# sparisi/pvr_habitat

Measured on AMD Instinct MI355X. Metric: frames/sec embedded (ResNet50, 256x256), higher is better.
Workload: dtype f16; 1 GPU; configs[1]: ResNet50 (MoCo-v2 layout) frozen, 256x256 uint8 frames resident in HBM, batch 256/GPU, random-init synthetic weights, f16 storage / MFMA inputs with fp32 accumulation (the product default, inside the 1e-3 parity bound; configs[1] names bf16); global_batch=256, frame=256, chunk=256, batches_in_flight=2, parallelism=frame shards, no collective (dp1)

## Files before the change

### pvr_habitat_amd/csrc/bottleneck_chain.hip

```cpp
#include "encoder_internal.h"

namespace pvr {


__device__ __forceinline__ void ch_dma16(__amdgpu_buffer_rsrc_t rs, char *lds, int voff, int soff) {
    __builtin_amdgcn_raw_ptr_buffer_load_lds(rs, (__attribute__((address_space(3))) void *)lds, 16, voff, soff, 0, 0);
}

#ifdef CHAIN_STAMP
__device__ unsigned long long chain_stamps[8192][12];
#define CH_T(i_) { if (threadIdx.x == 0) ch_tt[i_] = __builtin_amdgcn_s_memrealtime(); }
#else
#define CH_T(i_)
#endif

#ifndef CH_KNOCK
#define CH_KNOCK 0
#endif
template <int AUX = 0>
__device__ __forceinline__ void store_b128_imm(u32x4 v, __amdgpu_buffer_rsrc_t rs, int voff, int imm) {
    if constexpr (!(CH_KNOCK & 1)) __builtin_amdgcn_raw_buffer_store_b128(v, rs, voff + imm, 0, AUX);
}

template <int CM, int CMN, bool F16, int RD, int OCC, bool HALO, bool DS = false, int PFK = -1>
__global__ __launch_bounds__(256, OCC) void bottleneck_chain_kernel(ChainP p) {
    typedef typename HT<F16>::V8 V8;
    constexpr int BM = 128, BK = 64, BN = CM;
    constexpr int A_CH = BM / 32, B_CH = BN / 32, TM = 4, TN = BN / 32;
    constexpr int KS = CM / 64, HROWS = CM == 64 ? 256 : 192, RL = CM == 64 ? 3 : 2;
    constexpr int HSL = HROWS * 128, RING_OFF = KS * HSL, SLICE = CM * 128, ZERO_OFF = (HROWS - 1) * 128;
    constexpr int HOPS = KS * HROWS / 32;
    constexpr int STAGE = HALO ? (RING_OFF + 2 * SLICE) / 2 : (BM + BN) * 128;
    constexpr int C4 = 4 * CM, G = C4 / 64, KS3 = CM / 64;
    constexpr int TN1 = CMN / 32;
    constexpr int W3_CH = CM / 32, W1_CH = CMN / 32;
    constexpr int T2_OFF = 0;
    constexpr int YG_OFF = KS3 * 16384;
    constexpr int W3_OFF = YG_OFF + 16384;
    constexpr int W1_OFF = W3_OFF + KS3 * 8192;
    static_assert(W3_OFF + KS3 * 8192 <= 2 * STAGE, "phase-B tiles must fit the phase-A area");
    static_assert(RD >= 1 && RD <= G, "residual prefetch depth");
    extern __shared__ __attribute__((aligned(16))) char smem[];

    const int tid = threadIdx.x, lane = tid & 63, wave = tid >> 6;
#ifdef CHAIN_STAMP
    unsigned long long ch_tt[12] = {0, 0, 0, 0, 0, 0, 0, 0, 0, 0, 0, 0};
#endif
    CH_T(0);
    const int m0 = xcd_remap(blockIdx.x, gridDim.x) * BM;
    const int srow = tid >> 3, pch = tid & 7;
    const auto rs_in = __builtin_amdgcn_make_buffer_rsrc(const_cast<u16 *>(p.in), 0, p.in_bytes, 0x00020000);
    const auto rs_w2 = __builtin_amdgcn_make_buffer_rsrc(const_cast<u16 *>(p.w2), 0, p.w2_bytes, 0x00020000);
    const auto rs_w3 = __builtin_amdgcn_make_buffer_rsrc(const_cast<u16 *>(p.w3), 0, p.w3_bytes, 0x00020000);
    const auto rs_w1 = __builtin_amdgcn_make_buffer_rsrc(const_cast<u16 *>(p.w1n), 0, p.w1n_bytes, 0x00020000);
    const auto rs_res = __builtin_amdgcn_make_buffer_rsrc(const_cast<u16 *>(DS ? p.xds : p.res), 0, DS ? p.xds_bytes : p.y_bytes, 0x00020000);
    const auto rs_wd = __builtin_amdgcn_make_buffer_rsrc(const_cast<u16 *>(DS ? p.wds : p.w3), 0, DS ? p.wds_bytes : p.w3_bytes, 0x00020000);
    const auto rs_y = __builtin_amdgcn_make_buffer_rsrc(p.y, 0, p.y_bytes, 0x00020000);
    const auto rs_t = __builtin_amdgcn_make_buffer_rsrc(p.t1n, 0, p.t1n_bytes, 0x00020000);
// ... 64 lines not shown

    const int wm = wave >> 1, wn = wave & 1;
    const int fr = lane & 15, fq = lane >> 4;
    int x_rd[2][TM];
    int b_rd[2][TN];
#pragma unroll
    for (int ks = 0; ks < 2; ++ks) {
#pragma unroll
        for (int j = 0; j < TM; ++j) {
            const int row = wm * 64 + j * 16 + fr;
            x_rd[ks][j] = row * 128 + (((ks * 4 + fq) ^ ((row >> 1) & 7)) << 4);
        }
#pragma unroll
        for (int i = 0; i < TN; ++i) {
            const int row = wn * (BN / 2) + i * 16 + fr;
            b_rd[ks][i] = BM * 128 + row * 128 + (((ks * 4 + fq) ^ ((row >> 1) & 7)) << 4);
        }
    }

    const int y_nhwc = ((m0 + wm * 64 + fr) * C4 + wn * 32 + fq * 8) * 2;
    const int y_blkd = ((m0 >> 4) + wm * 4) * (C4 * 32) + (wn * 4 + fq) * 256 + fr * 16;
    const int y_off0 = p.y_blk ? y_blkd : y_nhwc, y_js = p.y_blk ? C4 * 32 : 16 * C4 * 2, y_gs = p.y_blk ? 2048 : 128;
    const int r_off0 = p.res_blk ? y_blkd : y_nhwc, r_js = p.res_blk ? C4 * 32 : 16 * C4 * 2, r_gs = p.res_blk ? 2048 : 128;
    const int t_nhwc = ((m0 + wm * 64 + fr) * CMN + wn * (CMN / 2) + fq * 8) * 2;
    const int t_blkd = ((m0 >> 4) + wm * 4) * (CMN * 32) + (wn * (CMN / 16) + fq) * 256 + fr * 16;
    const int t_off0 = p.t_blk ? t_blkd : t_nhwc, t_js = p.t_blk ? CMN * 32 : 16 * CMN * 2;
#define Y_OFF(j_) (y_off0 + (j_) * y_js)
#define R_OFF(j_) (r_off0 + (j_) * r_js)
#define T_OFF(j_) (t_off0 + (j_) * t_js)
    const int st_r = tid >> 3, st_c = ((tid & 7) ^ ((st_r >> 1) & 7)) * 16;
    const int w3_g0 = st_r * CM * 2 + st_c, w3_l0 = W3_OFF + st_r * 128 + (tid & 7) * 16;
    const int w1_g0 = st_r * C4 * 2 + st_c, w1_l0 = W1_OFF + st_r * 128 + (tid & 7) * 16;
#define W3_G(i_) (w3_g0 + ((i_) & 1) * (32 * CM * 2) + ((i_) >> 1) * 128)
#define W3_L(i_) (w3_l0 + ((i_) & 1) * 4096 + ((i_) >> 1) * 8192)
#define W1_G(i_) (w1_g0 + (i_) * (32 * C4 * 2))
#define W1_L(i_) (w1_l0 + (i_) * 4096)
    u32x4 rres[RD][TM], w3r[W3_CH], w1r[CMN ? W1_CH : 1];
#define PVR_PHASE_B_PREFETCH()                                                                                          \
    {                                                                                                                   \
        if constexpr (!DS) {                                                                                            \
            _Pragma("unroll") for (int d = 0; d < RD; ++d)                                                              \
                _Pragma("unroll") for (int j = 0; j < TM; ++j)                                                          \
                    rres[d][j] = __builtin_bit_cast(u32x4, __builtin_amdgcn_raw_buffer_load_b128(rs_res, (CH_KNOCK & 2) ? OOB : R_OFF(j), d * r_gs, DS ? 0 : PVR_NT_AUX(16))); \
        }                                                                                                               \
        _Pragma("unroll") for (int i = 0; i < W3_CH; ++i)                                                               \
            w3r[i] = __builtin_bit_cast(u32x4, __builtin_amdgcn_raw_buffer_load_b128(rs_w3, W3_G(i), 0, 0));            \
        if constexpr (CMN > 0) {                                                                                        \
// ... 125 lines not shown
        const int c = wn * (BN / 2) + i * 16 + fq * 4;
        const float4 bv = *reinterpret_cast<const float4 *>(p.b2 + c);
#pragma unroll
        for (int j = 0; j < TM; ++j) {
            const int row = wm * 64 + j * 16 + fr;
            const f32x4 a = acc2[i][j];
            const unsigned lo = pack2_h<F16>(fmaxf(a[0] + bv.x, 0.f), fmaxf(a[1] + bv.y, 0.f));
            const unsigned hi = pack2_h<F16>(fmaxf(a[2] + bv.z, 0.f), fmaxf(a[3] + bv.w, 0.f));
            const int cc = c & 63;
            char *dst = smem + T2_OFF + (c >> 6) * 16384 + row * 128 + ((((cc >> 3) ^ ((row >> 1) & 7))) << 4) + (cc & 4) * 2;
            *reinterpret_cast<uint2 *>(dst) = make_uint2(lo, hi);
        }
    }
#pragma unroll
    for (int i = 0; i < W3_CH; ++i) *reinterpret_cast<u32x4 *>(smem + W3_L(i)) = w3r[i];
    if constexpr (CMN > 0) {
#pragma unroll
        for (int i = 0; i < W1_CH; ++i) *reinterpret_cast<u32x4 *>(smem + W1_L(i)) = w1r[i];
    }
    if (G > 1) {
#pragma unroll
        for (int i = 0; i < W3_CH; ++i)
            w3r[i] = __builtin_bit_cast(u32x4, __builtin_amdgcn_raw_buffer_load_b128(rs_w3, W3_G(i), 64 * CM * 2, 0));
        if constexpr (CMN > 0) {
#pragma unroll
            for (int i = 0; i < W1_CH; ++i) w1r[i] = __builtin_bit_cast(u32x4, __builtin_amdgcn_raw_buffer_load_b128(rs_w1, W1_G(i), 128, 0));
        }
    }
    __syncthreads();
    CH_T(3);

    int w3_rd[2][2], w1_rd[2][CMN ? TN1 : 1], yg_wr[TM];
#pragma unroll
    for (int ks = 0; ks < 2; ++ks) {
#pragma unroll
        for (int t = 0; t < 2; ++t) {
            const int row = wn * 32 + t * 16 + fr;
            w3_rd[ks][t] = W3_OFF + row * 128 + (((ks * 4 + fq) ^ ((row >> 1) & 7)) << 4);
        }
        if constexpr (CMN > 0) {
#pragma unroll
            for (int i = 0; i < TN1; ++i) {
                const int row = wn * (CMN / 2) + i * 16 + fr;
                w1_rd[ks][i] = W1_OFF + row * 128 + (((ks * 4 + fq) ^ ((row >> 1) & 7)) << 4);
            }
        }
    }
#pragma unroll
    for (int j = 0; j < TM; ++j) {
        const int row = wm * 64 + j * 16 + fr;
        yg_wr[j] = YG_OFF + row * 128 + (((wn * 4 + fq) ^ ((row >> 1) & 7)) << 4);
    }
    f32x4 acc1[CMN ? TN1 : 1][TM];
    if constexpr (CMN > 0) {
#pragma unroll
        for (int i = 0; i < TN1; ++i)
#pragma unroll
            for (int j = 0; j < TM; ++j) acc1[i][j] = f32x4{0.f, 0.f, 0.f, 0.f};
    }

#pragma unroll
    for (int g = 0; g < G; ++g) {
        if (g == 1) CH_T(6);
        f32x4 acc3[2][TM];
#pragma unroll
        for (int t = 0; t < 2; ++t)
// ... 52 lines not shown
            if (p.y_blk) store_b128_imm<PVR_NT_AUX(4)>(o, rs_y, Y_OFF(j) + g * y_gs, 0);
            else store_b128_imm(o, rs_y, Y_OFF(j) + g * y_gs, 0);
            if constexpr (CMN > 0) *reinterpret_cast<u32x4 *>(smem + yg_wr[j]) = o;
        }
        if (!DS && g + RD < G) {
#pragma unroll
            for (int j = 0; j < TM; ++j)
                rres[g % RD][j] = __builtin_bit_cast(u32x4, __builtin_amdgcn_raw_buffer_load_b128(rs_res, (CH_KNOCK & 2) ? OOB : R_OFF(j), (g + RD) * r_gs, DS ? 0 : PVR_NT_AUX(16)));
        }
        if (g == 1) CH_T(8);
        __syncthreads();
        if (g == 1) CH_T(9);
        if (g + 1 < G) {
#pragma unroll
            for (int i = 0; i < W3_CH; ++i) *reinterpret_cast<u32x4 *>(smem + W3_L(i)) = w3r[i];
            if (g + 2 < G) {
#pragma unroll
                for (int i = 0; i < W3_CH; ++i)
                    w3r[i] = __builtin_bit_cast(u32x4, __builtin_amdgcn_raw_buffer_load_b128(rs_w3, W3_G(i), (g + 2) * (64 * CM * 2), 0));
            }
        }
        if (g == 1) CH_T(10);
        if constexpr (CMN == 0) __syncthreads();
        if constexpr (CMN > 0) {
#pragma unroll
            for (int ks = 0; ks < 2; ++ks) {
                V8 xa[TM], wb[TN1];
#pragma unroll
                for (int j = 0; j < TM; ++j) xa[j] = *reinterpret_cast<const V8 *>(smem + YG_OFF + x_rd[ks][j]);
#pragma unroll
                for (int i = 0; i < TN1; ++i) wb[i] = *reinterpret_cast<const V8 *>(smem + w1_rd[ks][i]);
#pragma unroll
                for (int i = 0; i < TN1; ++i)
#pragma unroll
                    for (int j = 0; j < TM; ++j) acc1[i][j] = mfma16<F16>(wb[i], xa[j], acc1[i][j]);
            }
            __syncthreads();
            if (g == 1) CH_T(11);
            if (g + 1 < G) {
#pragma unroll
                for (int i = 0; i < W1_CH; ++i) *reinterpret_cast<u32x4 *>(smem + W1_L(i)) = w1r[i];
                if (g + 2 < G) {
#pragma unroll
                    for (int i = 0; i < W1_CH; ++i)
                        w1r[i] = __builtin_bit_cast(u32x4, __builtin_amdgcn_raw_buffer_load_b128(rs_w1, W1_G(i), (g + 2) * 128, 0));
                }
            }
        }
    }

    CH_T(4);
    if constexpr (CMN > 0) {
#pragma unroll
        for (int q = 0; q < TN1 / 2; ++q) {
            const int c0 = wn * (CMN / 2) + q * 32 + fq * 8;
            const float4 bA = *reinterpret_cast<const float4 *>(p.b1n + c0), bB = *reinterpret_cast<const float4 *>(p.b1n + c0 + 4);
#pragma unroll
            for (int j = 0; j < TM; ++j) {
                const f32x4 lo = acc1[2 * q][j], hi = acc1[2 * q + 1][j];
                const float v[8] = {lo[0] + bA.x, lo[1] + bA.y, lo[2] + bA.z, lo[3] + bA.w, hi[0] + bB.x, hi[1] + bB.y, hi[2] + bB.z, hi[3] + bB.w};
                u32x4 o;
#pragma unroll
                for (int e = 0; e < 4; ++e)
                    o[e] = pack2_h<F16>(fmaxf(v[2 * e], 0.f), fmaxf(v[2 * e + 1], 0.f));
                if (p.t_blk) store_b128_imm<0>(o, rs_t, T_OFF(j) + q * 1024, 0);
                else store_b128_imm<PVR_NT_AUX(8)>(o, rs_t, T_OFF(j), q * 64);
            }
        }
    }
#undef PVR_PHASE_B_PREFETCH
#undef W3_G
#undef W3_L
#undef W1_G
#undef W1_L
#undef Y_OFF
#undef R_OFF
#undef T_OFF
#ifdef CHAIN_STAMP
    CH_T(5);
    if (threadIdx.x == 0 && blockIdx.x < 8192) { _Pragma("unroll") for (int k = 0; k < 12; ++k) chain_stamps[blockIdx.x][k] = ch_tt[k]; }
#endif
}

template <int CM, int CMN, bool F16, int RD, int OCC, bool HALO, bool DS = false, int PFK = -1>
static pvr_status launch_chain_one(ChainP &p, hipStream_t stream) {
    const int grid = (p.M + 127) / 128;
    const size_t pipe = HALO ? (size_t)(CM / 64) * (CM == 64 ? 256 : 192) * 128 + (size_t)2 * CM * 128 : (size_t)2 * (128 + CM) * 128;
    const size_t phase_b = (CM / 64) * 16384 + 16384 + (CM / 64) * 8192 + CMN * 128;
    const size_t lds = phase_b <= pipe ? pipe : phase_b;
    static DeviceOnce attr_done;
    if (attr_done.needed()) {
        PVR_HIP_TRY(hipFuncSetAttribute((const void *)bottleneck_chain_kernel<CM, CMN, F16, RD, OCC, HALO, DS, PFK>,
                                        hipFuncAttributeMaxDynamicSharedMemorySize, (int)lds));
        attr_done.mark();
    }
    hipLaunchKernelGGL((bottleneck_chain_kernel<CM, CMN, F16, RD, OCC, HALO, DS, PFK>), dim3(grid), dim3(256), lds, stream, p);
    PVR_LAUNCH_CHECK();
    return PVR_OK;
}

template <int CM, int CMN, bool F16, int RD, int OCC, bool DS = false>
static pvr_status launch_chain_inst(ChainP &p, const PlanSwitches &sw, hipStream_t stream) {
    const bool halo = p.stride == 1 && 128 + 2 * p.W + 2 <= (CM == 64 ? 256 : 192) - 1 && sw.chain_halo;
    if constexpr (DS) {
        if (halo) return sw.chain_ds_occ == 3 ? launch_chain_one<CM, CMN, F16, RD, 3, true, true>(p, stream) : launch_chain_one<CM, CMN, F16, RD, 2, true, true>(p, stream);
        return launch_chain_one<CM, CMN, F16, RD, 2, false, true>(p, stream);
    } else {
        if (halo) {
            if constexpr (CM == 128) {
                if (sw.chain_pfk == 12) return launch_chain_one<CM, CMN, F16, RD, 2, true, false, 12>(p, stream);
            }
            return launch_chain_one<CM, CMN, F16, RD, (CM == 64 ? OCC : 2), true>(p, stream);
        }
        return launch_chain_one<CM, CMN, F16, RD, OCC, false>(p, stream);
    }
}

template <bool F16>
static pvr_status launch_chain_dt(ChainP &p, int cm, int cmn, const PlanSwitches &sw, hipStream_t stream) {
    if (p.xds) {
        if (cm == 64 && cmn == 64) return launch_chain_inst<64, 64, F16, 1, 2, true>(p, sw, stream);
        set_error("bottleneck chain with downsample: no instance for Cm=%d, next Cm=%d", cm, cmn);
        return PVR_ERR_INVALID;
    }
    const int cfg = sw.chain_cfg;
#define PVR_CHAIN64(CMN_)                                                                 \
    switch (cfg) {                                                                        \
    case 12: return launch_chain_inst<64, CMN_, F16, 1, 2>(p, sw, stream);                \
    case 13: return launch_chain_inst<64, CMN_, F16, 1, 3>(p, sw, stream);                \
    case 22: return launch_chain_inst<64, CMN_, F16, 2, 2>(p, sw, stream);                \
    case 23: return launch_chain_inst<64, CMN_, F16, 2, 3>(p, sw, stream);                \
    default: return launch_chain_inst<64, CMN_, F16, 4, 2>(p, sw, stream);                \
    }
    if (cm == 64 && cmn == 64) PVR_CHAIN64(64)
    if (cm == 64 && cmn == 128) {
        if (cfg / 10 == 1) return launch_chain_inst<64, 128, F16, 1, 2>(p, sw, stream);
        if (cfg / 10 == 2) return launch_chain_inst<64, 128, F16, 2, 2>(p, sw, stream);
        return launch_chain_inst<64, 128, F16, 4, 2>(p, sw, stream);
    }
    if (cm == 64 && cmn == 0) PVR_CHAIN64(0)
#undef PVR_CHAIN64
    if (cm == 128 && cmn == 128) return launch_chain_inst<128, 128, F16, 1, 2>(p, sw, stream);
    if (cm == 128 && cmn == 0) return launch_chain_inst<128, 0, F16, 1, 2>(p, sw, stream);
    set_error("bottleneck chain: no instance for Cm=%d, next Cm=%d", cm, cmn);
    return PVR_ERR_INVALID;
}

bool chain_uses_wave_form(const PlanSwitches &sw, int cm, int cmn, int stride, bool ds) { return sw.chain_wave && chain_wave_supported(sw, cm, cmn, stride, ds); }

bool chain_uses_wave128(const PlanSwitches &sw, int cm, int cmn, int stride, int64_t M) { return sw.chain_wave && chain_wave128_supported(sw, cm, cmn, stride, M); }

bool chain_ds_supported(int cm, int cmn, int cin, int stride) { return cm == 64 && cmn == 64 && cin == 64 && stride == 1; }
bool chain_supported(int cm, int cmn) { return (cm == 64 && (cmn == 0 || cmn == 64 || cmn == 128)) || (cm == 128 && (cmn == 0 || cmn == 128)); }

int chain_row_source(int row) { return (row & ~31) + 8 * ((row >> 2) & 3) + 4 * ((row >> 4) & 1) + (row & 3); }

pvr_status launch_bottleneck_chain(const PlanSwitches &sw, const void *t1, const void *w2, const float *b2, const void *w3p, const float *b3, const void *res,
                                   void *y, const void *w1np, const float *b1n, void *t1n, int n, int h, int w, int cm, int cmn,
                                   int stride, int dtype, hipStream_t stream, const void *xds, const void *wdsp, const void *w3pb, const void *wdspb,
                                   int wave, int in_blk, int out_blk, const void *wpk, int y_s2) {
    PVR_REQUIRE(chain_supported(cm, cmn), "bottleneck chain: unsupported widths Cm=%d next=%d", cm, cmn);
    PVR_REQUIRE(t1 && w2 && b2 && w3p && b3 && (res || xds) && y && (cmn == 0 || (w1np && b1n && t1n)), "bottleneck chain: null argument");
    PVR_REQUIRE(!xds || (wdsp && chain_ds_supported(cm, cmn, 64, stride)), "bottleneck chain with downsample: unsupported shape");
    ChainP p;
    p.in = (const u16 *)t1; p.w2 = (const u16 *)w2; p.w3 = (const u16 *)w3p; p.w1n = (const u16 *)w1np; p.res = (const u16 *)res;
    p.b2 = b2; p.b3 = b3; p.b1n = b1n; p.y = (u16 *)y; p.t1n = (u16 *)t1n;
    p.N = n; p.H = h; p.W = w; p.stride = stride;
    p.Ho = (h + 2 - 3) / stride + 1; p.Wo = (w + 2 - 3) / stride + 1;
    const int64_t M = (int64_t)n * p.Ho * p.Wo;
    const int64_t inb = (int64_t)n * h * w * cm * 2, yb = M * 4 * cm * 2, tb = M * (cmn ? cmn : 1) * 2;
    PVR_REQUIRE(inb < 0x7ffffff0ll && yb < 0x7ffffff0ll && tb < 0x7ffffff0ll, "bottleneck chain: operand larger than 2 GiB (use a smaller chunk)");
    p.M = (int)M; p.in_bytes = (unsigned)inb; p.y_bytes = (unsigned)yb; p.t1n_bytes = (unsigned)tb;
    p.xds = (const u16 *)xds; p.wds = (const u16 *)wdsp;
    p.xds_bytes = xds ? (unsigned)(M * 64 * 2) : 0; p.wds_bytes = xds ? (unsigned)(4 * cm * 64 * 2) : 0;
    p.w2_bytes = (unsigned)(cm * 9 * cm * 2); p.w3_bytes = (unsigned)(4 * cm * cm * 2); p.w1n_bytes = (unsigned)(cmn * 4 * cm * 2);
    if (wave == 2) {
// ... 18 lines not shown
```

### pvr_habitat_amd/csrc/encoder.hip

```cpp
#include "encoder_internal.h"

namespace pvr {

pvr_status launch_split16_pack(const float *w, void *out, int rows, int K, hipStream_t stream);
bool conv_split16_supported(int cin, int cout, int k);
pvr_status launch_conv_split16(const float *in, const void *wsp, const float *bias, const float *res, float *out, int n, int h, int w, int cin,
                               int cout, int k, int stride, int pad, int relu, hipStream_t stream, float *out2 = nullptr, int n1 = 0, void *out16 = nullptr,
                               int terms = 3);

void read_switches(PlanSwitches &sw) {
    auto get = [](const char *name, int def) { const char *v = getenv(name); return v ? atoi(v) : def; };
    sw.pool_fuse = get("PVR_POOL_FUSE", 1);
    sw.stem_u8 = get("PVR_STEM_U8", 1);
    sw.stem_lds = get("PVR_STEM_LDS", 1);
    sw.stem_regpool = get("PVR_STEM_REGPOOL", 1);
    sw.frame_front1 = get("PVR_FRAME_FRONT1", 1);
    sw.frame_next1 = get("PVR_FRAME_NEXT1", 0);
    sw.frame_bneck = get("PVR_FRAME_BNECK", 1);
    sw.frame64 = get("PVR_FRAME64", 0);
    sw.bneck_stagger = get("PVR_FRAME_STAGGER", 0);
    sw.dual_ds = get("PVR_DUAL_DS", 1);
    sw.chain_ds = get("PVR_CHAIN_DS", 1);
    sw.chain_blocked = get("PVR_CHAIN_BLOCKED", 1);
    sw.chain_halo = get("PVR_CHAIN_HALO", 1);
    sw.chain_ds_occ = get("PVR_CHAIN_DS_OCC", 3);
    sw.chain_pfk = get("PVR_CHAIN_PFK", 12);
    sw.chain_cfg = get("PVR_CHAIN_CFG", 12);
    sw.chain_wave = get("PVR_CHAIN_WAVE", 1);
    sw.chain_wave_halo = get("PVR_CHAIN_WAVE_HALO", 1);
    sw.chain_wave_128 = get("PVR_CHAIN_WAVE_128", 1);
    sw.strided_y = get("PVR_STRIDED_Y", 1);
    sw.chain_wave_l2 = get("PVR_CHAIN_WAVE_L2", 0);
    sw.splitk = get("PVR_SPLITK", 1);
    sw.smallk_div = get("PVR_SMALLK_DIV", 4);
    if (sw.smallk_div < 1) sw.smallk_div = 1;
    sw.frame_min_n = get("PVR_FRAME_MIN_N", 128);
    sw.frame_run = get("PVR_FRAME_RUN", 0);
    sw.frame_stagger = get("PVR_FRAME_RUN_STAGGER", 0);
    sw.split16 = get("PVR_SPLIT16", 1);
    sw.stem_conv1 = get("PVR_STEM_CONV1", 1);
    sw.resid32 = get("PVR_RESID32", 1);
    sw.tail_f32 = get("PVR_TAIL_F32", 1);
    sw.fuse = get("PVR_FUSE", 1);
    sw.conv_algo = get("PVR_CONV_ALGO", -1);
    sw.conv_halo = get("PVR_CONV_HALO", 1);
    sw.conv_expand = get("PVR_CONV_EXPAND", 1);
    sw.conv_wfrag = get("PVR_CONV_WFRAG", 1);
    sw.wfrag_ko = get("PVR_WFRAG_KO", 0);
    sw.igemm_nk4 = get("PVR_IGEMM_NK4", 1);
    sw.igemm_bm64 = get("PVR_IGEMM_BM64", 0);
    sw.pp_bm224 = get("PVR_PP_BM224", 1);
    sw.pp_persist = get("PVR_PP_PERSIST", 384);
}

// ... 552 lines not shown
        const int a_cmn = e->ops[A.next1].cout;
        if (!e->sw.chain_blocked) continue;
        if (B.t1_in != A.t1_out || b3.res_buf != a3.out_buf || !a3.tap.empty() || b2.h != a2.h / a2.stride || b2.w != a2.w / a2.stride || b2.stride != 1) continue;
        if (B.wave == 2) {
            A.out_blk = A.wave == 2 ? 1 : 3; B.in_blk = 1;
            continue;
        }
        if (!A.wave && !B.wave) {
            if ((b2.h * b2.w) % 16 == 0) { A.out_blk = 1; B.in_blk = 1; }
            continue;
        }
        if (!A.wave || !B.wave) continue;
        if (!chain_wave_blocked_ok(a_cmn, a2.h, a2.w)) continue;
        A.out_blk = 1; B.in_blk = 1;
        if (A.ds >= 0 && a > 0 && a2.w == 56 && e->sw.chain_wave_halo) {
            Launch &C = e->sched_fused[a - 1];
            if (C.conv3 < 0 && C.conv2 >= 0) {
                const ConvOp &c1 = e->ops[C.conv2];
                if (c1.kind == 0 && !c1.f32op && c1.k == 1 && c1.stride == 1 && c1.out_buf == A.t1_in && c1.tap.empty() && c1.res_buf == B_NONE && !c1.out_f32 &&
                    c1.ksplit <= 1) { C.out_blk = 1; A.in_blk = 1; }
            }
        }
    }
    if (e->sw.stem_conv1 && !e->sched_fused.empty() && (e->desc.arch == PVR_ARCH_RESNET50 || e->desc.arch == PVR_ARCH_RESNET50_L3 || e->desc.arch == PVR_ARCH_RESNET50_L4)) {
        const Launch &L0 = e->sched_fused[0];
        if (L0.conv3 < 0 && L0.ds < 0 && L0.pair < 0 && !L0.frame && L0.conv2 == 0) {
            const ConvOp &c1 = e->ops[0];
            if (c1.kind == 0 && !c1.f32op && !c1.from32 && c1.k == 1 && c1.stride == 1 && c1.cin == 64 && c1.cout == 64 && c1.cin_real == 64 && c1.cout_real == 64 && c1.relu == 1 &&
                c1.in_buf == B_X0 && c1.out_buf == B_T1 && c1.res_buf == B_NONE && !c1.out_f32 && c1.tap.empty() && c1.ksplit <= 1 && c1.h == 56 && (int)c1.h_w.size() == 64 * 64) {
                std::vector<u16> img(64 * 64);
                stem_c1_pack(c1.h_w.data(), img.data());
                pvr_status s = enc_upload(&e->d_stem_c1w, img);
                if (s) return s;
                e->stem_c1 = 0; e->stem_c1_blk = L0.out_blk;
                e->sched_fused.erase(e->sched_fused.begin());
            }
        }
    }
    if (e->sw.strided_y) {
        std::vector<Launch> &sc = e->sched_fused;
        for (size_t a = 0; a < sc.size(); ++a) {
            Launch &A = sc[a];
            if (A.conv3 < 0 || A.frame || A.wave != 1 || A.next1 < 0 || A.ds >= 0) continue;
            const ConvOp &a2 = e->ops[A.conv2], &a3 = e->ops[A.conv3];
            if (a2.stride != 1 || !chain_wave_y_s2_ok(a2.cout, e->ops[A.next1].cout, a2.h, a2.w, A.out_blk)) continue;
            const int yb = a3.out_buf;
// ... 454 lines not shown
            } else
                s = launch_conv(enc->sw, enc->d_buf[c1.in_buf], c1.d_w, c1.d_b, nullptr, enc->d_buf[c1.out_buf], enc->d_zero, nb, c1.h, c1.w, c1.cin, c1.cout, 1, 1, 1, 0, c1.relu, 0, dt, st);
            if (s) return s;
        }
        bool pooled = false;
        const std::vector<Launch> &plan_ = cur_plan(enc);
        const uint8_t *kinds = enc->kinds.data() + (size_t)(nb - 1) * plan_.size();
        float *smallk = enc->d_smallk[enc->cur_lane];
        const bool pool_args_ok = enc->stop_after.empty() && out_stride % 4 == 0 && (((size_t)(out + (size_t)f0 * out_stride)) & 15) == 0;
        int launch_idx = 0;
        const bool run_ok = enc->stop_after.empty() && !enc->range_flags;
        const int stop_idx = enc->stop_after.size() > 1 && enc->stop_after[0] == '#' ? atoi(enc->stop_after.c_str() + 1) : -1;
        auto member = [&](const ConvOp &o, const void *in, const void *r_, void *out_) -> pvr_status {
            if (const int ks = small_batch_ksplit(enc, o, nb)) {
                if (!smallk) { set_error("low-latency plan without its scratch (pvr_encoder_set_low_latency allocates it)"); return PVR_ERR_STATE; }
                return launch_conv_splitk(in, o.d_w, o.d_b, r_, out_, enc->d_zero, smallk, ks, nb, o.h, o.w, o.cin, o.cout, o.k, o.k, o.stride, o.pad, o.relu, o.out_f32, dt, st);
            }
            return launch_conv(enc->sw, in, o.d_w, o.d_b, r_, out_, enc->d_zero, nb, o.h, o.w, o.cin, o.cout, o.k, o.k, o.stride, o.pad, o.relu, o.out_f32, dt, st);
        };
        for (size_t li = 0; li < plan_.size(); ++li) {
            const Launch &l = plan_[li];
            const ConvOp &op = enc->ops[l.conv3 >= 0 ? l.conv3 : l.conv2];
            const void *res = op.res_buf == B_NONE ? nullptr : enc->d_buf[op.res_buf];
            int kind = kinds[li];
            if (kind == LK_WFRAG_POOL && !pool_args_ok) kind = resolve_kind(enc, plan_, li, nb, false);
            if ((kind == LK_FRAME_RUN || kind == LK_FRAME_RUN_TAIL) && !run_ok) kind = LK_FRAME_FRONT1;
            if (kind == LK_CHAIN_YS2 && !run_ok) kind = LK_CHAIN;
            if (kind == LK_CONV_YS2 && !run_ok) kind = LK_CONV;
            switch (kind) {
            case LK_FRAME_RUN: {
                BFBlk blks[6];
                int nblk = 0;
                for (size_t t = li; t < plan_.size() && nblk < 6 && (t == li || kinds[t] == LK_FRAME_RUN_TAIL); ++t, ++nblk) {
                    const Launch &lt = plan_[t];
                    const ConvOp &o3 = enc->ops[lt.conv3], &o2 = enc->ops[lt.conv2], &o1 = enc->ops[lt.conv1];
                    blks[nblk] = BFBlk{(const u16 *)o1.d_wfb, (const u16 *)o2.d_wfb, (const u16 *)o3.d_wfb, (const u16 *)enc->d_buf[o3.res_buf], o1.d_b, o2.d_b, o3.d_b,
                                       (u16 *)enc->d_buf[o3.out_buf]};
                }
                s = launch_bneck_frame_run(blks, nblk, nb, dt, st, enc->sw.frame_stagger);
                break;
            }
            case LK_FRAME_RUN_TAIL:
                s = PVR_OK;
                break;
            case LK_FRAME_FRONT1: {
                const ConvOp &c2 = enc->ops[l.conv2], &cf = enc->ops[l.conv1];
// ... 2 lines not shown
                break;
            }
            case LK_FRAME: {
                const ConvOp &c2 = enc->ops[l.conv2];
                const ConvOp *c1 = l.next1 >= 0 ? &enc->ops[l.next1] : nullptr;
                s = launch_bneck_frame(enc->sw, enc->d_buf[l.t1_in], c2.d_wfb, c2.d_b, op.d_wfb, op.d_b, res, enc->d_buf[op.out_buf], nullptr, nb, c1 ? 7 : 3, dt, st,
                                       nullptr, c1 ? c1->d_wfb : nullptr, c1 ? c1->d_b : nullptr, c1 ? enc->d_buf[l.t1_out] : nullptr);
                break;
            }
            case LK_FRAME_MEMBERS: {
                const ConvOp &c2 = enc->ops[l.conv2];
                const ConvOp *c1 = l.next1 >= 0 ? &enc->ops[l.next1] : nullptr;
                const ConvOp *cf = l.conv1 >= 0 ? &enc->ops[l.conv1] : nullptr;
                const int t2b = l.t1_in == B_T1 ? B_T2 : B_T1;
                s = PVR_OK;
                if (cf) s = member(*cf, enc->d_buf[cf->in_buf], nullptr, enc->d_buf[l.t1_in]);
                if (!s) s = member(c2, enc->d_buf[l.t1_in], nullptr, enc->d_buf[t2b]);
                if (!s) s = member(op, enc->d_buf[t2b], res, enc->d_buf[op.out_buf]);
                if (!s && c1) s = member(*c1, enc->d_buf[op.out_buf], nullptr, enc->d_buf[l.t1_out]);
                break;
            }
            case LK_DUAL: {
                const ConvOp &cd = enc->ops[l.ds];
                s = launch_conv_pp256(enc->sw, enc->d_buf[op.in_buf], op.d_wcat, op.d_bsum, nullptr, enc->d_buf[op.out_buf], nb, op.h, op.w, op.cin, op.cout, 1, 1, 1, 0,
                                      op.relu, 0, 0, dt, 224, st, enc->d_buf[cd.in_buf], cd.h, cd.w, cd.cin, cd.stride);
                break;
            }
            case LK_DUAL_MEMBERS: {
                const ConvOp &cd = enc->ops[l.ds];
                s = member(cd, enc->d_buf[cd.in_buf], nullptr, enc->d_buf[cd.out_buf]);
                if (!s) s = member(op, enc->d_buf[op.in_buf], res, enc->d_buf[op.out_buf]);
                break;
            }
            case LK_CHAIN:
            case LK_CHAIN_YS2: {
                const ConvOp &c2 = enc->ops[l.conv2];
                const ConvOp *c1 = l.next1 >= 0 ? &enc->ops[l.next1] : nullptr;
                const ConvOp *cd = l.ds >= 0 ? &enc->ops[l.ds] : nullptr;
                s = launch_bottleneck_chain(enc->sw, enc->d_buf[l.t1_in], c2.d_w, c2.d_b, op.d_wp, cd ? op.d_bsum : op.d_b, res, enc->d_buf[op.out_buf],
                                            c1 ? c1->d_wp : nullptr, c1 ? c1->d_b : nullptr, c1 ? enc->d_buf[l.t1_out] : nullptr, nb,
                                            c2.h, c2.w, c2.cout, c1 ? c1->cout : 0, c2.stride, dt, st,
                                            cd ? enc->d_buf[cd->in_buf] : nullptr, cd ? cd->d_wp : nullptr, op.d_wpb, cd ? cd->d_wpb : nullptr,
                                            l.wave, cd ? (l.in_blk && t1_blocked) : l.in_blk, l.out_blk, c2.d_wpk, kind == LK_CHAIN_YS2);
                t1_blocked = false;
                break;
            }
            case LK_CONV_YS2:
                s = launch_conv_expand(enc->d_buf[op.in_buf], op.d_w, op.d_b, nullptr, enc->d_buf[op.out_buf], nb, op.h / 2, op.w / 2, op.cin, op.cout, 1, op.relu, dt, st);
                break;
            case LK_CAST:
                s = launch_f32_to_h((const float *)enc->d_buf[op.in_buf], enc->d_buf[op.out_buf], (size_t)nb * op.h * op.w * op.cin, dt, st);
                break;
            case LK_F32:
                s = launch_conv_f32((const float *)enc->d_buf[op.in_buf], op.d_wf, op.d_b, (const float *)res, (float *)enc->d_buf[op.out_buf], nb,
                                    op.h, op.w, op.cin, op.cout, op.k, op.stride, op.pad, op.relu, st);
                break;
            case LK_SPLIT16:
                s = launch_conv_split16((const float *)enc->d_buf[op.in_buf], op.d_wsp, op.d_b, (const float *)res, (float *)enc->d_buf[op.out_buf], nb,
                                        op.h, op.w, op.cin, op.cout, op.k, op.stride, op.pad, op.relu, st);
                break;
            case LK_SPLIT16_PAIR: {
                const ConvOp &od = enc->ops[l.pair];
                s = launch_conv_split16((const float *)enc->d_buf[op.in_buf], op.d_wsp_pair, op.d_b_pair, nullptr, (float *)enc->d_buf[op.out_buf], nb, op.h, op.w, op.cin,
                                        128, op.k, op.stride, op.pad, 1, st, (float *)enc->d_buf[od.out_buf], 64);
                break;
            }
            case LK_SPLIT16_IN32:
                s = launch_conv_split16((const float *)enc->d_buf[op.in_buf], op.d_wsp, op.d_b, nullptr, (op.out_f32 & 1) ? (float *)enc->d_buf[op.out_buf] : nullptr, nb,
                                        op.h, op.w, op.cin, op.cout, op.k, op.stride, op.pad, op.relu, st, nullptr, 0, (op.out_f32 & 1) ? nullptr : enc->d_buf[op.out_buf], 1);
                break;
            case LK_SPLITK_SMALL:
                s = member(op, enc->d_buf[op.in_buf], res, enc->d_buf[op.out_buf]);
                break;
            case LK_SPLITK:
                s = launch_conv_splitk(enc->d_buf[op.in_buf], op.d_w, op.d_b, res, enc->d_buf[op.out_buf], enc->d_zero, (float *)enc->d_buf[op.ks_buf],
                                       op.ksplit, nb, op.h, op.w, op.cin, op.cout, op.k, op.k, op.stride, op.pad, op.relu, op.out_f32, dt, st);
                break;
            case LK_EXPAND_BLOCKED:
                s = launch_conv_expand(enc->d_buf[op.in_buf], op.d_w, op.d_b, nullptr, enc->d_buf[op.out_buf], nb, op.h, op.w, op.cin, op.cout, 1, op.relu, dt, st, 1);
                t1_blocked = true;
                break;
            case LK_WFRAG_POOL:
                s = launch_conv_wfrag(enc->sw, enc->d_buf[op.in_buf], op.d_wfb, op.d_b, res, nullptr, nb, op.h, op.w, op.cin, op.cout, 1, 1, 1, 0, 1, 1, dt, st,
                                      out + (size_t)f0 * out_stride, out_stride);
                pooled = true;
                break;
            case LK_WFRAG:
                s = launch_conv_wfrag(enc->sw, enc->d_buf[op.in_buf], op.d_wfb, op.d_b, res, enc->d_buf[op.out_buf], nb, op.h, op.w, op.cin, op.cout, op.k, op.k,
                                      op.stride, op.pad, op.relu, op.out_f32, dt, st);
                break;
            default:
                s = launch_conv(enc->sw, enc->d_buf[op.in_buf], op.d_w, op.d_b, res, enc->d_buf[op.out_buf], enc->d_zero, nb, op.h, op.w,
                                op.cin, op.cout, op.k, op.k, op.stride, op.pad, op.relu, op.out_f32, dt, st);
            }
            if (s) return s;
            if (enc->range_flags && kind != LK_WFRAG_POOL) {
                const int ho_ = (op.h + 2 * op.pad - op.k) / op.stride + 1, wo_ = (op.w + 2 * op.pad - op.k) / op.stride + 1;
                const size_t n8 = (size_t)nb * ho_ * wo_ * op.cout / 8;
                const int blocks = (int)((n8 + 255) / 256 < 2048 ? (n8 + 255) / 256 : 2048);
                if ((op.out_f32 & 1) || op.f32op) hipLaunchKernelGGL(range_flag_kernel<true>, dim3(blocks), dim3(256), 0, st, enc->d_buf[op.out_buf], n8, dt, enc->range_flags, (int)li);
                else hipLaunchKernelGGL(range_flag_kernel<false>, dim3(blocks), dim3(256), 0, st, enc->d_buf[op.out_buf], n8, dt, enc->range_flags, (int)li);
            }
            if ((s = mark())) return s;
            if (!enc->stop_after.empty() && op.tap == enc->stop_after) { stopped = true; break; }
            if (launch_idx++ == stop_idx) { stopped = true; break; }
        }
        enc->last_pooled = pooled;
        if (stopped) return PVR_OK;
        float *o = out + (size_t)f0 * out_stride;
        if (pooled)
            s = PVR_OK;
        else if (pooled_head(enc))
            s = launch_avgpool(enc->d_buf[B_F32], o, out_stride, nb, enc->final_hw, enc->final_c, 1, dt, st);
        else
            s = launch_nhwc_to_chw((const float *)enc->d_buf[B_F32], o, out_stride, nb, enc->final_hw, enc->final_c,
                                   enc->final_creal, st);
        if (s) return s;
        if ((s = mark())) return s;
    }
    return PVR_OK;
}

static pvr_status lane_wait(pvr_encoder *enc, int lane, void *hip_stream) {
    hipStream_t st = (hipStream_t)hip_stream;
// ... 304 lines not shown
```

### pvr_habitat_amd/csrc/encoder_internal.h

```cpp
#pragma once
#include <map>
#include <string>
#include <vector>
#include <cmath>
#include "common.h"
#include "chain_params.h"

namespace pvr {

struct PlanSwitches {
    int pool_fuse = 1;
    int stem_u8 = 1;
    int stem_lds = 1;
    int stem_regpool = 1;
    int frame_front1 = 1;
    int frame_next1 = 0;
    int frame_bneck = 1;
    int frame64 = 0;
    int bneck_stagger = 0;
    int dual_ds = 1;
    int chain_ds = 1;
    int chain_blocked = 1;
    int chain_halo = 1;
    int chain_ds_occ = 3;
    int chain_pfk = 12;
    int chain_cfg = 12;
    int chain_wave = 1;
    int chain_wave_halo = 1;
    int chain_wave_128 = 1;
    int chain_wave_l2 = 0;
    int strided_y = 1;
    int splitk = 1;
    int smallk_div = 4;
    int frame_run = 0;
    int frame_stagger = 0;
    int frame_min_n = 128;
    int stem_conv1 = 1;
    int split16 = 1;
    int resid32 = 1;
    int tail_f32 = 1;
    int fuse = 1;
    int conv_algo = -1;
    int conv_halo = 1;
    int conv_expand = 1;
    int conv_wfrag = 1;
    int wfrag_ko = 0;
    int igemm_nk4 = 1;
    int igemm_bm64 = 0;
    int pp_bm224 = 1;
    int pp_persist = 384;
};
void read_switches(PlanSwitches &sw);
PlanSwitches &op_switches();

// ... 206 lines not shown
```

Baseline: 100,200 frames/s.

## Fuse stage-boundary conv1 (Cmn=256) into the preceding bottleneck chain kernel

Adds a Cm=128, Cmn=256 instance of the bottleneck chain kernel. It computes the next stage's first 1x1 conv (256 outputs) in two halves of 128, so the weight tile fits in LDS. A new schedule pass fuses that boundary conv1 into the previous block's chain launch and remaps the t1 buffers for the following launches. The goal is to drop one launch and one round trip of the 512-channel activation through HBM. The cost is extra syncs and weight reloads per output group, and the halo pfk=12 path is disabled for this instance.

```diff
diff --git a/pvr_habitat_amd/csrc/bottleneck_chain.hip b/pvr_habitat_amd/csrc/bottleneck_chain.hip
--- a/pvr_habitat_amd/csrc/bottleneck_chain.hip
+++ b/pvr_habitat_amd/csrc/bottleneck_chain.hip
@@ -16,6 +16,9 @@
 
 #ifndef CH_KNOCK
 #define CH_KNOCK 0
+#endif
+#ifndef CH_W1_AHEAD
+#define CH_W1_AHEAD 0
 #endif
 template <int AUX = 0>
 __device__ __forceinline__ void store_b128_imm(u32x4 v, __amdgpu_buffer_rsrc_t rs, int voff, int imm) {
@@ -33,7 +36,8 @@
     constexpr int STAGE = HALO ? (RING_OFF + 2 * SLICE) / 2 : (BM + BN) * 128;
     constexpr int C4 = 4 * CM, G = C4 / 64, KS3 = CM / 64;
     constexpr int TN1 = CMN / 32;
-    constexpr int W3_CH = CM / 32, W1_CH = CMN / 32;
+    constexpr int NH = CMN > 128 ? 2 : 1, CMH = CMN / NH, TNW = CMH / 32;
+    constexpr int W3_CH = CM / 32, W1_CH = CMH / 32;
     constexpr int T2_OFF = 0;
     constexpr int YG_OFF = KS3 * 16384;
     constexpr int W3_OFF = YG_OFF + 16384;
@@ -144,7 +148,7 @@
     const int y_blkd = ((m0 >> 4) + wm * 4) * (C4 * 32) + (wn * 4 + fq) * 256 + fr * 16;
     const int y_off0 = p.y_blk ? y_blkd : y_nhwc, y_js = p.y_blk ? C4 * 32 : 16 * C4 * 2, y_gs = p.y_blk ? 2048 : 128;
     const int r_off0 = p.res_blk ? y_blkd : y_nhwc, r_js = p.res_blk ? C4 * 32 : 16 * C4 * 2, r_gs = p.res_blk ? 2048 : 128;
-    const int t_nhwc = ((m0 + wm * 64 + fr) * CMN + wn * (CMN / 2) + fq * 8) * 2;
+    const int t_nhwc = ((m0 + wm * 64 + fr) * CMN + wn * (CMH / 2) + fq * 8) * 2;
     const int t_blkd = ((m0 >> 4) + wm * 4) * (CMN * 32) + (wn * (CMN / 16) + fq) * 256 + fr * 16;
     const int t_off0 = p.t_blk ? t_blkd : t_nhwc, t_js = p.t_blk ? CMN * 32 : 16 * CMN * 2;
 #define Y_OFF(j_) (y_off0 + (j_) * y_js)
@@ -316,15 +320,15 @@
 #pragma unroll
         for (int i = 0; i < W3_CH; ++i)
             w3r[i] = __builtin_bit_cast(u32x4, __builtin_amdgcn_raw_buffer_load_b128(rs_w3, W3_G(i), 64 * CM * 2, 0));
-        if constexpr (CMN > 0) {
-#pragma unroll
-            for (int i = 0; i < W1_CH; ++i) w1r[i] = __builtin_bit_cast(u32x4, __builtin_amdgcn_raw_buffer_load_b128(rs_w1, W1_G(i), 128, 0));
+        if constexpr (CMN > 0 && (NH == 1 || CH_W1_AHEAD)) {
+#pragma unroll
+            for (int i = 0; i < W1_CH; ++i) w1r[i] = __builtin_bit_cast(u32x4, __builtin_amdgcn_raw_buffer_load_b128(rs_w1, W1_G(i), NH == 2 ? CMH * C4 * 2 : 128, 0));
         }
     }
     __syncthreads();
     CH_T(3);
 
-    int w3_rd[2][2], w1_rd[2][CMN ? TN1 : 1], yg_wr[TM];
+    int w3_rd[2][2], w1_rd[2][CMN ? TNW : 1], yg_wr[TM];
 #pragma unroll
     for (int ks = 0; ks < 2; ++ks) {
 #pragma unroll
@@ -334,8 +338,8 @@
         }
         if constexpr (CMN > 0) {
 #pragma unroll
-            for (int i = 0; i < TN1; ++i) {
-                const int row = wn * (CMN / 2) + i * 16 + fr;
+            for (int i = 0; i < TNW; ++i) {
+                const int row = wn * (CMH / 2) + i * 16 + fr;
                 w1_rd[ks][i] = W1_OFF + row * 128 + (((ks * 4 + fq) ^ ((row >> 1) & 7)) << 4);
             }
         }
@@ -434,7 +438,44 @@
         }
         if (g == 1) CH_T(10);
         if constexpr (CMN == 0) __syncthreads();
-        if constexpr (CMN > 0) {
+        if constexpr (NH == 2) {
+#pragma unroll
+            for (int h = 0; h < 2; ++h) {
+                if (h == 1) __syncthreads();
+                if (!CH_W1_AHEAD && (h == 0 || g + 1 < G)) {
+#pragma unroll
+                    for (int i = 0; i < W1_CH; ++i)
+                        w1r[i] = __builtin_bit_cast(u32x4, __builtin_amdgcn_raw_buffer_load_b128(rs_w1, W1_G(i), (g + h) * 128 + (1 - h) * (CMH * C4 * 2), 0));
+                }
+#pragma unroll
+                for (int ks = 0; ks < 2; ++ks) {
+                    V8 xa[TM];
+#pragma unroll
+                    for (int j = 0; j < TM; ++j) xa[j] = *reinterpret_cast<const V8 *>(smem + YG_OFF + x_rd[ks][j]);
+#pragma unroll
+                    for (int ip = 0; ip < TNW; ip += 2) {
+                        V8 wb[2];
+#pragma unroll
+                        for (int i = 0; i < 2; ++i) wb[i] = *reinterpret_cast<const V8 *>(smem + w1_rd[ks][ip + i]);
+#pragma unroll
+                        for (int i = 0; i < 2; ++i)
+#pragma unroll
+                            for (int j = 0; j < TM; ++j) acc1[h * TNW + ip + i][j] = mfma16<F16>(wb[i], xa[j], acc1[h * TNW + ip + i][j]);
+                    }
+                }
+                __syncthreads();
+                if (h == 0 || g + 1 < G) {
+#pragma unroll
+                    for (int i = 0; i < W1_CH; ++i) *reinterpret_cast<u32x4 *>(smem + W1_L(i)) = w1r[i];
+                    if (CH_W1_AHEAD && g + 1 < G) {
+#pragma unroll
+                        for (int i = 0; i < W1_CH; ++i)
+                            w1r[i] = __builtin_bit_cast(u32x4, __builtin_amdgcn_raw_buffer_load_b128(rs_w1, W1_G(i), (g + 1) * 128 + h * (CMH * C4 * 2), 0));
+                    }
+                }
+            }
+        }
+        if constexpr (CMN > 0 && NH == 1) {
 #pragma unroll
             for (int ks = 0; ks < 2; ++ks) {
                 V8 xa[TM], wb[TN1];
@@ -465,7 +506,8 @@
     if constexpr (CMN > 0) {
 #pragma unroll
         for (int q = 0; q < TN1 / 2; ++q) {
-            const int c0 = wn * (CMN / 2) + q * 32 + fq * 8;
+            constexpr int QH = TNW / 2;
+            const int c0 = (q / QH) * CMH + wn * (CMH / 2) + (q % QH) * 32 + fq * 8;
             const float4 bA = *reinterpret_cast<const float4 *>(p.b1n + c0), bB = *reinterpret_cast<const float4 *>(p.b1n + c0 + 4);
 #pragma unroll
             for (int j = 0; j < TM; ++j) {
@@ -476,7 +518,7 @@
                 for (int e = 0; e < 4; ++e)
                     o[e] = pack2_h<F16>(fmaxf(v[2 * e], 0.f), fmaxf(v[2 * e + 1], 0.f));
                 if (p.t_blk) store_b128_imm<0>(o, rs_t, T_OFF(j) + q * 1024, 0);
-                else store_b128_imm<PVR_NT_AUX(8)>(o, rs_t, T_OFF(j), q * 64);
+                else store_b128_imm<PVR_NT_AUX(8)>(o, rs_t, T_OFF(j), (q / QH) * (CMH * 2) + (q % QH) * 64);
             }
         }
     }
@@ -498,7 +540,7 @@
 static pvr_status launch_chain_one(ChainP &p, hipStream_t stream) {
     const int grid = (p.M + 127) / 128;
     const size_t pipe = HALO ? (size_t)(CM / 64) * (CM == 64 ? 256 : 192) * 128 + (size_t)2 * CM * 128 : (size_t)2 * (128 + CM) * 128;
-    const size_t phase_b = (CM / 64) * 16384 + 16384 + (CM / 64) * 8192 + CMN * 128;
+    const size_t phase_b = (CM / 64) * 16384 + 16384 + (CM / 64) * 8192 + (CMN > 128 ? CMN / 2 : CMN) * 128;
     const size_t lds = phase_b <= pipe ? pipe : phase_b;
     static DeviceOnce attr_done;
     if (attr_done.needed()) {
@@ -519,7 +561,7 @@
         return launch_chain_one<CM, CMN, F16, RD, 2, false, true>(p, stream);
     } else {
         if (halo) {
-            if constexpr (CM == 128) {
+            if constexpr (CM == 128 && CMN <= 128) {
                 if (sw.chain_pfk == 12) return launch_chain_one<CM, CMN, F16, RD, 2, true, false, 12>(p, stream);
             }
             return launch_chain_one<CM, CMN, F16, RD, (CM == 64 ? OCC : 2), true>(p, stream);
@@ -554,6 +596,10 @@
 #undef PVR_CHAIN64
     if (cm == 128 && cmn == 128) return launch_chain_inst<128, 128, F16, 1, 2>(p, sw, stream);
     if (cm == 128 && cmn == 0) return launch_chain_inst<128, 0, F16, 1, 2>(p, sw, stream);
+    if (cm == 128 && cmn == 256) {
+        PVR_REQUIRE(!p.t_blk, "bottleneck chain: the Cmn = 256 instance writes t1' in NHWC only");
+        return launch_chain_inst<128, 256, F16, 1, 2>(p, sw, stream);
+    }
     set_error("bottleneck chain: no instance for Cm=%d, next Cm=%d", cm, cmn);
     return PVR_ERR_INVALID;
 }
@@ -563,7 +609,7 @@
 bool chain_uses_wave128(const PlanSwitches &sw, int cm, int cmn, int stride, int64_t M) { return sw.chain_wave && chain_wave128_supported(sw, cm, cmn, stride, M); }
 
 bool chain_ds_supported(int cm, int cmn, int cin, int stride) { return cm == 64 && cmn == 64 && cin == 64 && stride == 1; }
-bool chain_supported(int cm, int cmn) { return (cm == 64 && (cmn == 0 || cmn == 64 || cmn == 128)) || (cm == 128 && (cmn == 0 || cmn == 128)); }
+bool chain_supported(int cm, int cmn) { return (cm == 64 && (cmn == 0 || cmn == 64 || cmn == 128)) || (cm == 128 && (cmn == 0 || cmn == 128 || cmn == 256)); }
 
 int chain_row_source(int row) { return (row & ~31) + 8 * ((row >> 2) & 3) + 4 * ((row >> 4) & 1) + (row & 3); }
 
diff --git a/pvr_habitat_amd/csrc/encoder.hip b/pvr_habitat_amd/csrc/encoder.hip
--- a/pvr_habitat_amd/csrc/encoder.hip
+++ b/pvr_habitat_amd/csrc/encoder.hip
@@ -30,6 +30,7 @@
     sw.chain_wave_halo = get("PVR_CHAIN_WAVE_HALO", 1);
     sw.chain_wave_128 = get("PVR_CHAIN_WAVE_128", 1);
     sw.strided_y = get("PVR_STRIDED_Y", 1);
+    sw.boundary_conv1 = get("PVR_BOUNDARY_CONV1", 1);
     sw.chain_wave_l2 = get("PVR_CHAIN_WAVE_L2", 0);
     sw.splitk = get("PVR_SPLITK", 1);
     sw.smallk_div = get("PVR_SMALLK_DIV", 4);
@@ -628,6 +629,40 @@
             }
         }
     }
+    if (e->sw.boundary_conv1) {
+        std::vector<Launch> &sc = e->sched_fused;
+        auto plain = [](const Launch &l) { return l.conv3 < 0 && l.ds < 0 && l.pair < 0 && !l.frame && l.conv1 < 0 && l.next1 < 0 && !l.in_blk && !l.out_blk; };
+        auto t1buf = [](int b) { return b == B_T1 || b == B_T2; };
+        for (size_t a = 0; a + 3 < sc.size(); ++a) {
+            Launch &A = sc[a], &Cl = sc[a + 2], &D = sc[a + 3];
+            const Launch &B = sc[a + 1];
+            if (A.conv3 < 0 || A.frame || A.wave || A.next1 >= 0 || A.ds >= 0 || A.out_blk || !t1buf(A.t1_in)) continue;
+            if (!plain(B) || !plain(Cl) || D.conv3 >= 0 || D.ds < 0 || D.frame || B.conv2 != A.conv3 + 1 || Cl.conv2 != B.conv2 + 1) continue;
+            const ConvOp &a2 = e->ops[A.conv2], &a3 = e->ops[A.conv3], &c2 = e->ops[Cl.conv2], &d3 = e->ops[D.conv2], &dd = e->ops[D.ds];
+            ConvOp &c1 = e->ops[B.conv2];
+            if (a2.stride != 1 || a2.cout != 128 || c1.cout != 256 || !chain_supported(a2.cout, c1.cout) || a3.out_f32) continue;
+            if (!ends_with(c1.conv, ".conv1") || c1.kind != 0 || c1.f32op || c1.from32 || c1.k != 1 || c1.stride != 1 || c1.pad != 0 || c1.relu != 1 || c1.out_f32 ||
+                c1.res_buf != B_NONE || !c1.tap.empty() || c1.ksplit > 1 || c1.cin != 4 * a2.cout || c1.cin_real != c1.cin || c1.cout_real != c1.cout ||
+                c1.in_buf != a3.out_buf || c1.h != a2.h || c1.w != a2.w || !t1buf(c1.out_buf) || c1.h_w.size() != (size_t)c1.cout * c1.cin)
+                continue;
+            if (c2.kind != 0 || c2.f32op || c2.from32 || c2.k != 3 || c2.in_buf != c1.out_buf || c2.res_buf != B_NONE || c2.out_f32 || !c2.tap.empty() || c2.ksplit > 1 ||
+                !t1buf(c2.out_buf) || c2.out_buf == c2.in_buf || d3.in_buf != c2.out_buf || dd.in_buf != a3.out_buf)
+                continue;
+            if (!c1.d_wp) {
+                const size_t K = (size_t)c1.cin;
+                std::vector<u16> hp((size_t)c1.cout * K);
+                for (int r = 0; r < c1.cout; ++r) memcpy(&hp[(size_t)r * K], &c1.h_w[(size_t)chain_row_source(r) * K], K * 2);
+                pvr_status s = enc_upload(&c1.d_wp, hp);
+                if (s) return s;
+            }
+            A.next1 = B.conv2;
+            A.t1_out = A.t1_in == B_T1 ? B_T2 : B_T1;
+            Cl.t1_in = A.t1_out; Cl.t1_out = A.t1_in;
+            D.t1_in = Cl.t1_out;
+            sc.erase(sc.begin() + a + 1);
+            break;
+        }
+    }
     if (e->sw.stem_conv1 && !e->sched_fused.empty() && (e->desc.arch == PVR_ARCH_RESNET50 || e->desc.arch == PVR_ARCH_RESNET50_L3 || e->desc.arch == PVR_ARCH_RESNET50_L4)) {
         const Launch &L0 = e->sched_fused[0];
         if (L0.conv3 < 0 && L0.ds < 0 && L0.pair < 0 && !L0.frame && L0.conv2 == 0) {
@@ -1128,6 +1163,7 @@
             const Launch &l = plan_[li];
             const ConvOp &op = enc->ops[l.conv3 >= 0 ? l.conv3 : l.conv2];
             const void *res = op.res_buf == B_NONE ? nullptr : enc->d_buf[op.res_buf];
+            const int in_b = l.conv3 < 0 && l.t1_in != B_NONE ? l.t1_in : op.in_buf, out_b = l.conv3 < 0 && l.t1_out != B_NONE ? l.t1_out : op.out_buf;
             int kind = kinds[li];
             if (kind == LK_WFRAG_POOL && !pool_args_ok) kind = resolve_kind(enc, plan_, li, nb, false);
             if ((kind == LK_FRAME_RUN || kind == LK_FRAME_RUN_TAIL) && !run_ok) kind = LK_FRAME_FRONT1;
@@ -1176,14 +1212,14 @@
             }
             case LK_DUAL: {
                 const ConvOp &cd = enc->ops[l.ds];
-                s = launch_conv_pp256(enc->sw, enc->d_buf[op.in_buf], op.d_wcat, op.d_bsum, nullptr, enc->d_buf[op.out_buf], nb, op.h, op.w, op.cin, op.cout, 1, 1, 1, 0,
+                s = launch_conv_pp256(enc->sw, enc->d_buf[in_b], op.d_wcat, op.d_bsum, nullptr, enc->d_buf[out_b], nb, op.h, op.w, op.cin, op.cout, 1, 1, 1, 0,
                                       op.relu, 0, 0, dt, 224, st, enc->d_buf[cd.in_buf], cd.h, cd.w, cd.cin, cd.stride);
                 break;
             }
             case LK_DUAL_MEMBERS: {
                 const ConvOp &cd = enc->ops[l.ds];
                 s = member(cd, enc->d_buf[cd.in_buf], nullptr, enc->d_buf[cd.out_buf]);
-                if (!s) s = member(op, enc->d_buf[op.in_buf], res, enc->d_buf[op.out_buf]);
+                if (!s) s = member(op, enc->d_buf[in_b], res, enc->d_buf[out_b]);
                 break;
             }
             case LK_CHAIN:
@@ -1224,7 +1260,7 @@
                                         op.h, op.w, op.cin, op.cout, op.k, op.stride, op.pad, op.relu, st, nullptr, 0, (op.out_f32 & 1) ? nullptr : enc->d_buf[op.out_buf], 1);
                 break;
             case LK_SPLITK_SMALL:
-                s = member(op, enc->d_buf[op.in_buf], res, enc->d_buf[op.out_buf]);
+                s = member(op, enc->d_buf[in_b], res, enc->d_buf[out_b]);
                 break;
             case LK_SPLITK:
                 s = launch_conv_splitk(enc->d_buf[op.in_buf], op.d_w, op.d_b, res, enc->d_buf[op.out_buf], enc->d_zero, (float *)enc->d_buf[op.ks_buf],
@@ -1240,11 +1276,11 @@
                 pooled = true;
                 break;
             case LK_WFRAG:
-                s = launch_conv_wfrag(enc->sw, enc->d_buf[op.in_buf], op.d_wfb, op.d_b, res, enc->d_buf[op.out_buf], nb, op.h, op.w, op.cin, op.cout, op.k, op.k,
+                s = launch_conv_wfrag(enc->sw, enc->d_buf[in_b], op.d_wfb, op.d_b, res, enc->d_buf[out_b], nb, op.h, op.w, op.cin, op.cout, op.k, op.k,
                                       op.stride, op.pad, op.relu, op.out_f32, dt, st);
                 break;
             default:
-                s = launch_conv(enc->sw, enc->d_buf[op.in_buf], op.d_w, op.d_b, res, enc->d_buf[op.out_buf], enc->d_zero, nb, op.h, op.w,
+                s = launch_conv(enc->sw, enc->d_buf[in_b], op.d_w, op.d_b, res, enc->d_buf[out_b], enc->d_zero, nb, op.h, op.w,
                                 op.cin, op.cout, op.k, op.k, op.stride, op.pad, op.relu, op.out_f32, dt, st);
             }
             if (s) return s;
@@ -1252,8 +1288,8 @@
                 const int ho_ = (op.h + 2 * op.pad - op.k) / op.stride + 1, wo_ = (op.w + 2 * op.pad - op.k) / op.stride + 1;
                 const size_t n8 = (size_t)nb * ho_ * wo_ * op.cout / 8;
                 const int blocks = (int)((n8 + 255) / 256 < 2048 ? (n8 + 255) / 256 : 2048);
-                if ((op.out_f32 & 1) || op.f32op) hipLaunchKernelGGL(range_flag_kernel<true>, dim3(blocks), dim3(256), 0, st, enc->d_buf[op.out_buf], n8, dt, enc->range_flags, (int)li);
-                else hipLaunchKernelGGL(range_flag_kernel<false>, dim3(blocks), dim3(256), 0, st, enc->d_buf[op.out_buf], n8, dt, enc->range_flags, (int)li);
+                if ((op.out_f32 & 1) || op.f32op) hipLaunchKernelGGL(range_flag_kernel<true>, dim3(blocks), dim3(256), 0, st, enc->d_buf[out_b], n8, dt, enc->range_flags, (int)li);
+                else hipLaunchKernelGGL(range_flag_kernel<false>, dim3(blocks), dim3(256), 0, st, enc->d_buf[out_b], n8, dt, enc->range_flags, (int)li);
             }
             if ((s = mark())) return s;
             if (!enc->stop_after.empty() && op.tap == enc->stop_after) { stopped = true; break; }
diff --git a/pvr_habitat_amd/csrc/encoder_internal.h b/pvr_habitat_amd/csrc/encoder_internal.h
--- a/pvr_habitat_amd/csrc/encoder_internal.h
+++ b/pvr_habitat_amd/csrc/encoder_internal.h
@@ -30,6 +30,7 @@
     int chain_wave_128 = 1;
     int chain_wave_l2 = 0;
     int strided_y = 1;
+    int boundary_conv1 = 1;
     int splitk = 1;
     int smallk_div = 4;
     int frame_run = 0;
```

Result: no change. 99820 frames/s (-0.3%).
